# kan-bayashi/ParallelWaveGAN

Measured on AMD Instinct MI355X. Metric: HiFi-GAN V1 22.05 kHz generator inference RTF^-1 (audio samples/s), higher is better.
Workload: dtype f32; 1 GPU; HiFi-GAN V1 generator fwd, LJSpeech 22.05 kHz, B16 x 800 mel frames per GPU, fp32, random init; global_batch=16, parallelism=replicas x1

## Files before the change

### include/pwg_kernels.h

```cpp
#ifndef PWG_KERNELS_H_
#define PWG_KERNELS_H_

#include <stddef.h>
#include <stdint.h>

#ifdef __cplusplus
extern "C" {
#endif

typedef enum pwg_status {
  PWG_OK = 0,
  PWG_ERR_BAD_SHAPE = -1,
  PWG_ERR_UNSUPPORTED = -2,
  PWG_ERR_LAUNCH = -3,
  PWG_ERR_NULL = -4,
  PWG_ERR_WORKSPACE = -5
} pwg_status;

const char* pwg_last_error(void);
int pwg_abi_version(void);
int pwg_target_arch(void);

int pwg_prof_enable(int on);
int pwg_prof_reset(void);
// ... 72 lines not shown
int pwg_conv1d_num_tile_configs(void);
int pwg_conv1d_forward_cfg(const pwg_conv1d_desc* d, const float* x, const float* w_packed,
                           const float* bias, const float* add1, const float* add2, float* y,
                           int32_t tile_config, int32_t use_dma, void* stream);

int pwg_conv1d_bf16_supported(const pwg_conv1d_desc* d);
size_t pwg_conv1d_bf16_packed_weight_bytes(const pwg_conv1d_desc* d);
int pwg_conv1d_bf16_pack_weight(const pwg_conv1d_desc* d, const float* w, const float* scale, void* w_packed,
                                void* stream);
int pwg_conv1d_bf16_forward(const pwg_conv1d_desc* d, const float* x, const void* w_packed, const float* bias,
                            const float* add1, const float* add2, float* y, float* workspace, size_t workspace_floats,
                            void* stream);
int pwg_conv1d_bf16_forward_cfg(const pwg_conv1d_desc* d, const float* x, const void* w_packed, const float* bias,
                                const float* add1, const float* add2, float* y, int32_t mfma_shape, void* stream);

int pwg_conv1d_split_supported(const pwg_conv1d_desc* d);
size_t pwg_conv1d_split_packed_weight_bytes(const pwg_conv1d_desc* d);
int pwg_conv1d_split_pack_weight(const pwg_conv1d_desc* d, const float* w, const float* scale, void* w_packed,
                                 void* stream);
int pwg_conv1d_split_forward(const pwg_conv1d_desc* d, const float* x, const void* w_packed, const float* bias,
                             const float* add1, const float* add2, float* y, float* workspace, size_t workspace_floats,
                             void* stream);
int pwg_conv1d_split_forward_cfg(const pwg_conv1d_desc* d, const float* x, const void* w_packed, const float* bias,
                                 const float* add1, const float* add2, float* y, int32_t mfma_shape, int32_t tile_mode,
                                 void* stream);
int pwg_conv1d_split_step_form(const pwg_conv1d_desc* d);
int pwg_conv1d_split_forward_step(const pwg_conv1d_desc* d, const float* x, const void* w_packed, const float* bias,
                                  const float* add1, const float* add2, float* y, int32_t mfma_shape, int32_t tile_mode,
                                  int32_t step_form, void* stream);
int pwg_conv1d_split_window_form(const pwg_conv1d_desc* d);
int pwg_conv1d_split_forward_window(const pwg_conv1d_desc* d, const float* x, const void* w_packed, const float* bias,
                                    const float* add1, const float* add2, float* y, int32_t mfma_shape,
                                    int32_t tile_mode, int32_t step_form, int32_t window_form, void* stream);

int pwg_convtr1d_split_supported(const pwg_conv1d_desc* d);
size_t pwg_convtr1d_split_packed_weight_bytes(const pwg_conv1d_desc* d);
int pwg_convtr1d_split_pack_weight(const pwg_conv1d_desc* d, const float* w, const float* scale, void* w_packed,
                                   void* stream);
int pwg_convtr1d_split_forward(const pwg_conv1d_desc* d, const float* x, const void* w_packed, const float* bias,
                               const float* add1, const float* add2, float* y, float* workspace,
                               size_t workspace_floats, void* stream);
int pwg_convtr1d_split_forward_cfg(const pwg_conv1d_desc* d, const float* x, const void* w_packed, const float* bias,
                                   const float* add1, const float* add2, float* y, int32_t mfma_shape,
                                   int32_t tile_mode, void* stream);

int pwg_conv1d_stream_supported(const pwg_conv1d_desc* d);
size_t pwg_conv1d_stream_hist_floats(const pwg_conv1d_desc* d);
int pwg_conv1d_stream_forward(const pwg_conv1d_desc* d, const float* x, const float* hist_in, float* hist_out,
                              const float* w_packed, const float* bias, const float* add1, const float* add2, float* y,
                              void* stream);

int pwg_conv1d_stream_bf16_supported(const pwg_conv1d_desc* d);
int pwg_conv1d_stream_bf16_forward(const pwg_conv1d_desc* d, const float* x, const float* hist_in, float* hist_out,
                                   const void* w_packed_bf16, const float* bias, const float* add1,
                                   const float* add2, float* y, void* stream);

int pwg_conv1d_stream_delayed_supported(const pwg_conv1d_desc* d, int32_t delay1, int32_t delay2);
int pwg_conv1d_stream_delayed_forward(const pwg_conv1d_desc* d, const float* x, const float* hist_in, float* hist_out,
                                      const float* w_packed, const float* bias, const float* add1,
                                      const float* add1_hist_in, float* add1_hist_out, int32_t delay1, const float* add2,
                                      const float* add2_hist_in, float* add2_hist_out, int32_t delay2, int32_t valid_lo,
                                      int32_t valid_hi, float* y, void* stream);

int pwg_conv1d_stream_bf16_delayed_supported(const pwg_conv1d_desc* d, int32_t delay1, int32_t delay2);
int pwg_conv1d_stream_bf16_delayed_forward(const pwg_conv1d_desc* d, const float* x, const float* hist_in,
                                           float* hist_out, const void* w_packed_bf16, const float* bias,
// ... 359 lines not shown
```

### parallelwavegan_amd/_lib.py

```python
import ctypes
import os

_HERE = os.path.dirname(os.path.abspath(__file__))
LIB_PATH = os.environ.get("PWG_KERNEL_LIB") or os.path.join(_HERE, "libpwgkernels.so")

PWG_ACT_NONE, PWG_ACT_LEAKY_RELU, PWG_ACT_TANH, PWG_ACT_RELU = 0, 1, 2, 3
PWG_PAD_ZERO, PWG_PAD_REFLECT, PWG_PAD_REPLICATE = 0, 1, 2
ABI_VERSION = 15
SPECTRAL_NORM_SCRATCH_FLOATS = 257


class ConvDesc(ctypes.Structure):

    _fields_ = [
        ("batch", ctypes.c_int32),
        ("c_in", ctypes.c_int32),
        ("c_out", ctypes.c_int32),
        ("t_in", ctypes.c_int32),
        ("t_out", ctypes.c_int32),
        ("width", ctypes.c_int32),
        ("kernel", ctypes.c_int32),
        ("stride", ctypes.c_int32),
        ("dilation", ctypes.c_int32),
        ("pad_left", ctypes.c_int32),
# ... 82 lines not shown
    "pwg_target_arch": (ctypes.c_int, []),
    "pwg_debug_poison_lds": (ctypes.c_int, [ctypes.c_int]),
    "pwg_set_concurrency_hint": (ctypes.c_float, [ctypes.c_float]),
    "pwg_prof_enable": (ctypes.c_int, [ctypes.c_int]),
    "pwg_prof_reset": (ctypes.c_int, []),
    "pwg_prof_num_kernels": (ctypes.c_int, []),
    "pwg_prof_get": (ctypes.c_int, [_i32, ctypes.c_char_p, ctypes.c_size_t, ctypes.POINTER(ctypes.c_double),
                                    ctypes.POINTER(ctypes.c_int64), ctypes.POINTER(ctypes.c_double),
                                    ctypes.POINTER(ctypes.c_double)]),
    "pwg_conv1d_packed_weight_floats": (ctypes.c_size_t, [ctypes.POINTER(ConvDesc)]),
    "pwg_conv1d_pack_weight": (ctypes.c_int, [ctypes.POINTER(ConvDesc), _vp, _vp, _vp, _vp]),
    "pwg_conv1d_forward_workspace_floats": (ctypes.c_size_t, [ctypes.POINTER(ConvDesc)]),
    "pwg_conv1d_forward": (ctypes.c_int, [ctypes.POINTER(ConvDesc), _vp, _vp, _vp, _vp, _vp, _vp, _vp, ctypes.c_size_t,
                                          _vp]),
    "pwg_conv1d_bf16_supported": (ctypes.c_int, [ctypes.POINTER(ConvDesc)]),
    "pwg_conv1d_bf16_packed_weight_bytes": (ctypes.c_size_t, [ctypes.POINTER(ConvDesc)]),
    "pwg_conv1d_bf16_pack_weight": (ctypes.c_int, [ctypes.POINTER(ConvDesc), _vp, _vp, _vp, _vp]),
    "pwg_conv1d_bf16_forward": (ctypes.c_int, [ctypes.POINTER(ConvDesc), _vp, _vp, _vp, _vp, _vp, _vp, _vp, ctypes.c_size_t,
                                               _vp]),
    "pwg_conv1d_bf16_forward_cfg": (ctypes.c_int, [ctypes.POINTER(ConvDesc), _vp, _vp, _vp, _vp, _vp, _vp, _i32, _vp]),
    "pwg_conv1d_split_supported": (ctypes.c_int, [ctypes.POINTER(ConvDesc)]),
    "pwg_conv1d_split_packed_weight_bytes": (ctypes.c_size_t, [ctypes.POINTER(ConvDesc)]),
    "pwg_conv1d_split_pack_weight": (ctypes.c_int, [ctypes.POINTER(ConvDesc), _vp, _vp, _vp, _vp]),
    "pwg_conv1d_split_forward": (ctypes.c_int, [ctypes.POINTER(ConvDesc), _vp, _vp, _vp, _vp, _vp, _vp, _vp,
                                                ctypes.c_size_t, _vp]),
    "pwg_conv1d_split_forward_cfg": (ctypes.c_int, [ctypes.POINTER(ConvDesc), _vp, _vp, _vp, _vp, _vp, _vp, _i32, _i32,
                                                    _vp]),
    "pwg_conv1d_split_step_form": (ctypes.c_int, [ctypes.POINTER(ConvDesc)]),
    "pwg_conv1d_split_forward_step": (ctypes.c_int, [ctypes.POINTER(ConvDesc), _vp, _vp, _vp, _vp, _vp, _vp, _i32, _i32,
                                                     _i32, _vp]),
    "pwg_conv1d_split_window_form": (ctypes.c_int, [ctypes.POINTER(ConvDesc)]),
    "pwg_conv1d_split_forward_window": (ctypes.c_int, [ctypes.POINTER(ConvDesc), _vp, _vp, _vp, _vp, _vp, _vp, _i32,
                                                       _i32, _i32, _i32, _vp]),
    "pwg_convtr1d_split_supported": (ctypes.c_int, [ctypes.POINTER(ConvDesc)]),
    "pwg_convtr1d_split_packed_weight_bytes": (ctypes.c_size_t, [ctypes.POINTER(ConvDesc)]),
    "pwg_convtr1d_split_pack_weight": (ctypes.c_int, [ctypes.POINTER(ConvDesc), _vp, _vp, _vp, _vp]),
    "pwg_convtr1d_split_forward": (ctypes.c_int, [ctypes.POINTER(ConvDesc), _vp, _vp, _vp, _vp, _vp, _vp, _vp,
                                                  ctypes.c_size_t, _vp]),
    "pwg_convtr1d_split_forward_cfg": (ctypes.c_int, [ctypes.POINTER(ConvDesc), _vp, _vp, _vp, _vp, _vp, _vp, _i32, _i32,
                                                      _vp]),
    "pwg_conv1d_stream_supported": (ctypes.c_int, [ctypes.POINTER(ConvDesc)]),
    "pwg_conv1d_stream_hist_floats": (ctypes.c_size_t, [ctypes.POINTER(ConvDesc)]),
    "pwg_conv1d_stream_forward": (ctypes.c_int, [ctypes.POINTER(ConvDesc), _vp, _vp, _vp, _vp, _vp, _vp, _vp, _vp, _vp]),
    "pwg_conv1d_stream_bf16_supported": (ctypes.c_int, [ctypes.POINTER(ConvDesc)]),
    "pwg_conv1d_stream_bf16_forward": (ctypes.c_int, [ctypes.POINTER(ConvDesc), _vp, _vp, _vp, _vp, _vp, _vp, _vp, _vp,
                                                      _vp]),
    "pwg_conv1d_stream_delayed_supported": (ctypes.c_int, [ctypes.POINTER(ConvDesc), _i32, _i32]),
    "pwg_conv1d_stream_delayed_forward": (ctypes.c_int, [ctypes.POINTER(ConvDesc), _vp, _vp, _vp, _vp, _vp, _vp, _vp, _vp,
                                                         _i32, _vp, _vp, _vp, _i32, _i32, _i32, _vp, _vp]),
    "pwg_conv1d_stream_bf16_delayed_supported": (ctypes.c_int, [ctypes.POINTER(ConvDesc), _i32, _i32]),
    "pwg_conv1d_stream_bf16_delayed_forward": (ctypes.c_int, [ctypes.POINTER(ConvDesc), _vp, _vp, _vp, _vp, _vp, _vp, _vp,
                                                              _vp, _i32, _vp, _vp, _vp, _i32, _i32, _i32, _vp, _vp]),
    "pwg_conv1d_stream_slots_forward": (ctypes.c_int, [ctypes.POINTER(ConvDesc), _vp, _vp, _vp, _vp, _vp, _vp, _vp, _vp,
                                                       _i32, _vp, _vp, _vp, _i32, _vp, _i32, _i32, _vp, _vp]),
    "pwg_conv1d_stream_slots_forward_bf16": (ctypes.c_int, [ctypes.POINTER(ConvDesc), _vp, _vp, _vp, _vp, _vp, _vp, _vp,
                                                            _vp, _i32, _vp, _vp, _vp, _i32, _vp, _i32, _i32, _vp, _vp]),
    "pwg_conv1d_stream_mirrored_supported": (ctypes.c_int, [ctypes.POINTER(ConvDesc)]),
    "pwg_conv1d_stream_mirrored_forward": (ctypes.c_int, [ctypes.POINTER(ConvDesc), _vp, _vp, _vp, _vp, _vp, _vp, _i32,
                                                          _i32, _i32, _i32, _vp]),
    "pwg_conv1d_packed_weight_bwd_floats": (ctypes.c_size_t, [ctypes.POINTER(ConvDesc)]),
    "pwg_conv1d_pack_weight_bwd": (ctypes.c_int, [ctypes.POINTER(ConvDesc), _vp, _vp, _vp, _vp]),
    "pwg_weight_bank_table_bytes": (ctypes.c_size_t, [_i32]),
    "pwg_weight_bank_build": (ctypes.c_int, [ctypes.POINTER(BankItem), _i32, _vp, ctypes.c_size_t,
                                             ctypes.POINTER(ctypes.c_int32)]),
    "pwg_weight_bank_prepare": (ctypes.c_int, [_vp, ctypes.POINTER(ctypes.c_int32), _i32, _vp]),
    "pwg_conv1d_backward_data_workspace_floats": (ctypes.c_size_t, [ctypes.POINTER(ConvDesc)]),
# ... 177 lines not shown
```

### parallelwavegan_amd/csrc/conv1d_split.hip

```cpp
#include "mfma_conv.h"

namespace pwg {
namespace {

constexpr int PARTS = 3;

struct SplitArgs : MfmaConvArgs {
  int plane;
  long part_stride;
  float pre_mul;
  unsigned pre_mask;
  int wide_out;
};

static int split_geometry(const pwg_conv1d_desc* d, MfmaConvGeom* g) {
  return mfma_conv_geometry("conv1d_split", PARTS, false, d, g);
}

__device__ __forceinline__ float pre_activate(float v, float mul, unsigned mask) {
  const float n = __uint_as_float(__float_as_uint(v * mul) & mask);
  return v > 0.f ? v : n;
}

template <int NT, bool CHECKED>
// ... 7 lines not shown
    const int t = base + grp * 4;
    const float* __restrict__ src = xc + (size_t)(oct * 8) * a.t_in + t;
    if (!CHECKED) {
      if (grp < ngroups) {
#pragma unroll
        for (int j = 0; j < 8; ++j) st[it][j] = *reinterpret_cast<const f32x4*>(src + (size_t)j * a.t_in);
      }
    } else {
      const bool tin = grp < ngroups && t >= 0 && t < a.t_in;
#pragma unroll
      for (int j = 0; j < 8; ++j) {
        f32x4 v = {0.f, 0.f, 0.f, 0.f};
        if (tin && oct * 8 + j < c_left) v = *reinterpret_cast<const f32x4*>(src + (size_t)j * a.t_in);
        st[it][j] = v;
      }
    }
  }
#pragma unroll
  for (int it = 0; it < ITEMS; ++it) {
    const int idx = tid + it * 256, oct = idx & 3, grp = idx >> 2;
    if (grp < ngroups) {
#pragma unroll
      for (int e = 0; e < 4; ++e) {
        float v[8];
#pragma unroll
        for (int j = 0; j < 8; ++j) v[j] = pre_activate(st[it][j][e], a.pre_mul, a.pre_mask);
        split3_store<8>(v, xs + (grp * 4 + e) * kConvRow + oct * 8, a.plane);
        __builtin_amdgcn_sched_barrier(0);
      }
    }
  }
}

template <int TILE, int TM, int TN, bool WIDE, bool FULL>
__device__ __forceinline__ void split_epilogue(const SplitArgs& a, const typename Mfma<TILE>::acc_t (&acc)[TM][TN],
                                               int row0, int col0, size_t out_base) {
  constexpr int HL = 64 / TILE, NG = TILE * TILE / 64 / 4, NV = TN * NG;
  constexpr int NB = WIDE ? NV : 1, BATCHES = TM * NV / NB;
  const bool has_bias = a.bias != nullptr, has1 = a.add1 != nullptr, has2 = a.add2 != nullptr;
#pragma unroll
  for (int bi = 0; bi < BATCHES; ++bi) {
    const int mi = bi * NB / NV;
    const int m = row0 + mi * TILE, mc = FULL ? m : min(m, a.m - 1);
    const size_t row = out_base + (size_t)mc * a.t_out;
    int q[NB];
#pragma unroll
    for (int k = 0; k < NB; ++k) {
      const int n = (bi * NB + k) % NV;
      q[k] = col0 + (n / NG) * TILE + (n % NG) * (4 * HL);
    }
    auto load = [&](const float* __restrict__ src, f32x4 (&t)[NB]) {
#pragma unroll
      for (int k = 0; k < NB; ++k) {
        if (WIDE) {
          t[k] = *reinterpret_cast<const f32x4*>(src + row + (FULL ? q[k] : min(q[k], a.nq - 4)));
        } else {
#pragma unroll
          for (int e = 0; e < 4; ++e) t[k][e] = src[row + min(q[k] + e, a.nq - 1)];
        }
      }
    };
    f32x4 t1[NB], t2[NB], v[NB];
    float bias = 0.f;
    if (has_bias) bias = a.bias[mc];
    if (has1) load(a.add1, t1);
    if (has2) load(a.add2, t2);
#pragma unroll
    for (int k = 0; k < NB; ++k) {
      const int n = (bi * NB + k) % NV;
#pragma unroll
      for (int e = 0; e < 4; ++e) v[k][e] = acc[mi][n / NG][(n % NG) * 4 + e];
// ... 189 lines not shown
#pragma unroll
  for (int mi = 0; mi < TM; ++mi)
#pragma unroll
    for (int ni = 0; ni < TN; ++ni)
#pragma unroll
      for (int i = 0; i < NREG; ++i) acc[mi][ni][i] = 0.f;

  for (int chunk = 0; chunk < a.cin_chunks; ++chunk) {
    if (chunk) __syncthreads();
    stage_chunk<NT, VEC>(a, c, chunk, xs);
    __syncthreads();
#pragma unroll 1
    for (int s = 0; s < a.taps * KSTEPS; ++s) {
      const SplitStepId next = split_step_successor(step, a.cin_chunks, a.taps, KSTEPS);
      split_step_streamed<TILE, TM, TN, kConvRow, true>(
          wf, a.w, a.part_stride, wrow + split_step_rows<TILE>(a.cin_chunks, a.m_pad, step, c.h),
          wrow + split_step_rows<TILE>(a.cin_chunks, a.m_pad, next, c.h), xs,
          c.sh + c.wave_n * (WN * 32) + c.r + step.tap * a.dil, split_step_off<TILE>(step, c.h), a.plane, acc);
      step = next;
    }
  }

  const size_t out_base = (size_t)c.b * a.c_out * a.t_out;
  const int row0 = c.m0 + c.wave_m * (WM * 32) + c.r, col0 = c.q0 + c.wave_n * (WN * 32) + 4 * c.h;
  const bool full = c.m0 + MT <= a.m && c.q0 + NT <= a.nq;
  if (!a.wide_out)
    split_epilogue<TILE, TM, TN, false, false>(a, acc, row0, col0, out_base);
  else if (full)
    split_epilogue<TILE, TM, TN, true, true>(a, acc, row0, col0, out_base);
  else
    split_epilogue<TILE, TM, TN, true, false>(a, acc, row0, col0, out_base);
}

typedef __attribute__((address_space(3))) void* lds_ptr_t;

static inline size_t split_raw_bytes(int rows) { return (size_t)KC * rows * sizeof(float); }

__device__ __forceinline__ void request_raw_window(const float* __restrict__ xw, int t_in, int ngroups, float* raww,
                                                   int lane) {
  const int total = 8 * ngroups;
  const int dq = 64 / ngroups, dr = 64 - dq * ngroups;
  int j = lane / ngroups, g = lane - j * ngroups;
  for (int e0 = 0; e0 < total; e0 += 64) {
    if (e0 + lane < total)
      __builtin_amdgcn_global_load_lds(xw + (size_t)j * t_in + 4 * g, (lds_ptr_t)(raww + e0 * 4), 16, 0, 0);
    j += dq, g += dr;
    if (g >= ngroups) g -= ngroups, ++j;
  }
}

__device__ __forceinline__ void split_raw_window(const SplitArgs& a, const float* raww, int ngroups, __bf16* xs, int wave,
                                                 int lane) {
  for (int grp = lane; grp < ngroups; grp += 64) {
    f32x4 st[8];
#pragma unroll
    for (int j = 0; j < 8; ++j) st[j] = *reinterpret_cast<const f32x4*>(raww + (j * ngroups + grp) * 4);
#pragma unroll
    for (int e = 0; e < 4; ++e) {
      float v[8];
#pragma unroll
      for (int j = 0; j < 8; ++j) v[j] = pre_activate(st[j][e], a.pre_mul, a.pre_mask);
      split3_store<8>(v, xs + (grp * 4 + e) * kConvRow + wave * 8, a.plane);
      __builtin_amdgcn_sched_barrier(0);
    }
  }
}
// ... 79 lines not shown
  };
};

static void split_fill_args(SplitArgs* a, const pwg_conv1d_desc* d, const MfmaConvGeom& g, const MfmaConvPlan& p,
                            const float* x, const void* w_packed, const float* bias, const float* add1, const float* add2,
                            float* y) {
  mfma_conv_fill_args(a, d, g, x, w_packed, bias, add1, add2, y);
  a->plane = p.plane;
  a->part_stride = image_elems(g) / 8;
  a->pre_mul = d->pre_act == PWG_ACT_LEAKY_RELU ? d->pre_slope : (d->pre_act == PWG_ACT_RELU ? 0.0f : 1.0f);
  a->pre_mask = d->pre_act == PWG_ACT_RELU ? 0u : ~0u;
  a->wide_out = d->t_out % 4 == 0 && ((reinterpret_cast<uintptr_t>(y) | reinterpret_cast<uintptr_t>(add1) |
                                       reinterpret_cast<uintptr_t>(add2)) & 15u) == 0;
}

constexpr int kStepPlanDecides = 0, kStepResident = 1, kStepStreamed = 2;
constexpr int kStreamedMinTaps = 7, kStreamedMinChunks = 2;
static int split_step_form(const MfmaConvGeom& g) {
  if (!split_image_addressable(image_elems(g))) return kStepResident;
  return g.taps >= kStreamedMinTaps && g.cin_chunks >= kStreamedMinChunks ? kStepStreamed : kStepResident;
}

constexpr int kWindowPlanDecides = 0, kWindowStaged = 1, kWindowPrefetched = 2;
constexpr size_t kLdsPerCu = 160 * 1024, kWindowLdsShare = kLdsPerCu / 3;
constexpr int kWindowMaxTaps = 0;
static size_t split_window_lds(const MfmaConvPlan& p) { return p.lds + split_raw_bytes(p.plane / kConvRow); }
static bool split_window_covers(const MfmaConvPlan& p) { return p.vec && split_window_lds(p) <= kLdsPerCu; }
static int split_window_form(const MfmaConvGeom& g, const MfmaConvPlan& p) {
  if (!split_window_covers(p) || split_step_form(g) == kStepStreamed) return kWindowStaged;
  return g.taps <= kWindowMaxTaps && g.cin_chunks >= 2 && split_window_lds(p) <= kWindowLdsShare ? kWindowPrefetched
                                                                                                   : kWindowStaged;
}

static int split_forward(const pwg_conv1d_desc* d, const float* x, const void* w_packed, const float* bias,
                         const float* add1, const float* add2, float* y, int mfma_shape, int tile_mode, int step_form,
                         int window_form, hipStream_t stream) {
  MfmaConvGeom g;
  int rc = split_geometry(d, &g);
  if (rc != PWG_OK) return rc;
  PWG_REQUIRE(step_form >= kStepPlanDecides && step_form <= kStepStreamed, PWG_ERR_BAD_SHAPE,
              "conv1d_split: step_form = %d (0 = the plan decides, 1 = resident, 2 = streamed)", step_form);
  PWG_REQUIRE(window_form >= kWindowPlanDecides && window_form <= kWindowPrefetched, PWG_ERR_BAD_SHAPE,
              "conv1d_split: window_form = %d (0 = the plan decides, 1 = staged, 2 = prefetched)", window_form);
  rc = mfma_conv_check_forward("conv1d_split", d, x, w_packed, y, mfma_shape, tile_mode);
  if (rc != PWG_OK) return rc;
  const MfmaConvPlan p = mfma_conv_plan(d, g, PARTS, tile_mode, x, add1, add2);
  PWG_REQUIRE(step_form != kStepStreamed || split_image_addressable(image_elems(g)), PWG_ERR_UNSUPPORTED,
              "conv1d_split: weight image too large for the streamed step");
  PWG_REQUIRE(window_form != kWindowPrefetched || step_form != kStepStreamed, PWG_ERR_UNSUPPORTED,
              "conv1d_split: the prefetched window (window_form = 2) has no streamed step (step_form = 2)");
  PWG_REQUIRE(window_form != kWindowPrefetched || p.vec, PWG_ERR_UNSUPPORTED,
              "conv1d_split: the prefetched window (window_form = 2) needs 16-B staging: t_in %% 4 == 0, x 16-B aligned, "
              "a window of at most %d columns", 2 * p.nt);
  PWG_REQUIRE(window_form != kWindowPrefetched || split_window_covers(p), PWG_ERR_UNSUPPORTED,
              "conv1d_split: the prefetched window (window_form = 2) needs %zu B of LDS (> %zu)", split_window_lds(p),
              kLdsPerCu);
  const bool prefetched = window_form == kWindowPrefetched ||
                          (window_form == kWindowPlanDecides && step_form == kStepPlanDecides &&
                           split_window_form(g, p) == kWindowPrefetched);
  const bool streamed = !prefetched && (step_form == kStepPlanDecides ? split_step_form(g) : step_form) == kStepStreamed;
  SplitArgs a;
  split_fill_args(&a, d, g, p, x, w_packed, bias, add1, add2, y);
  if (prefetched) {
    const size_t lds = split_window_lds(p);
    void (*kern)(SplitArgs) = mfma_shape == 32 ? mfma_conv_tile_kernel<WindowFamily::K, 32, SplitArgs>(p)
                                               : mfma_conv_tile_kernel<WindowFamily::K, 16, SplitArgs>(p);
    if (lds > kConvMaxLds && !lds_limit_is_set(reinterpret_cast<const void*>(kern), lds)) {
      hipError_t e = hipFuncSetAttribute(reinterpret_cast<const void*>(kern), hipFuncAttributeMaxDynamicSharedMemorySize,
                                         (int)lds);
      PWG_REQUIRE(e == hipSuccess, PWG_ERR_LAUNCH, "conv1d_split: cannot raise LDS limit to %zu: %s", lds,
                  hipGetErrorString(e));
    }
    maybe_poison_lds(stream);
    ProfScope prof(stream, "conv1d_split_mfma_kernel", p.flops, p.bytes);
    hipLaunchKernelGGL(kern, p.grid, dim3(256), lds, stream, a);
    PWG_CHECK_LAUNCH("conv1d_split");
    return PWG_OK;
  }
  maybe_poison_lds(stream);
  ProfScope prof(stream, "conv1d_split_mfma_kernel", p.flops, p.bytes);
  if (p.vec) {
    if (streamed)
      mfma_conv_launch<Family<true, true>::K>(p, mfma_shape, a, stream);
    else
      mfma_conv_launch<Family<true, false>::K>(p, mfma_shape, a, stream);
  } else {
    if (streamed)
      mfma_conv_launch<Family<false, true>::K>(p, mfma_shape, a, stream);
    else
      mfma_conv_launch<Family<false, false>::K>(p, mfma_shape, a, stream);
  }
  PWG_CHECK_LAUNCH("conv1d_split");
  return PWG_OK;
}

// ... 217 lines not shown
}
}

using namespace pwg;

extern "C" int pwg_conv1d_split_supported(const pwg_conv1d_desc* d) {
  MfmaConvGeom g;
  return split_geometry(d, &g) == PWG_OK ? 1 : 0;
}

extern "C" size_t pwg_conv1d_split_packed_weight_bytes(const pwg_conv1d_desc* d) {
  MfmaConvGeom g;
  if (split_geometry(d, &g) != PWG_OK) return 0;
  return (size_t)PARTS * image_elems(g) * sizeof(__bf16);
}

extern "C" int pwg_conv1d_split_pack_weight(const pwg_conv1d_desc* d, const float* w, const float* scale, void* w_packed,
                                            void* stream) {
  MfmaConvGeom g;
  int rc = split_geometry(d, &g);
  if (rc != PWG_OK) return rc;
  PWG_REQUIRE(w && w_packed, PWG_ERR_NULL, "conv1d_split_pack_weight: NULL pointer");
  mfma_conv_pack<PARTS>(d, g, w, scale, w_packed, (hipStream_t)stream);
  PWG_CHECK_LAUNCH("conv1d_split_pack_weight");
  return PWG_OK;
}

extern "C" int pwg_conv1d_split_forward(const pwg_conv1d_desc* d, const float* x, const void* w_packed, const float* bias,
                                        const float* add1, const float* add2, float* y, float* workspace,
                                        size_t workspace_floats, void* stream) {
  (void)workspace;
  (void)workspace_floats;
  return split_forward(d, x, w_packed, bias, add1, add2, y, kDefaultMfmaShape, 0, kStepPlanDecides, kWindowPlanDecides,
                       (hipStream_t)stream);
}

extern "C" int pwg_conv1d_split_forward_cfg(const pwg_conv1d_desc* d, const float* x, const void* w_packed,
                                            const float* bias, const float* add1, const float* add2, float* y,
                                            int32_t mfma_shape, int32_t tile_mode, void* stream) {
  return split_forward(d, x, w_packed, bias, add1, add2, y, mfma_shape, tile_mode, kStepPlanDecides, kWindowPlanDecides,
                       (hipStream_t)stream);
}

extern "C" int pwg_conv1d_split_forward_step(const pwg_conv1d_desc* d, const float* x, const void* w_packed,
                                             const float* bias, const float* add1, const float* add2, float* y,
                                             int32_t mfma_shape, int32_t tile_mode, int32_t step_form, void* stream) {
  return split_forward(d, x, w_packed, bias, add1, add2, y, mfma_shape, tile_mode, step_form, kWindowPlanDecides,
                       (hipStream_t)stream);
}

extern "C" int pwg_conv1d_split_forward_window(const pwg_conv1d_desc* d, const float* x, const void* w_packed,
                                               const float* bias, const float* add1, const float* add2, float* y,
                                               int32_t mfma_shape, int32_t tile_mode, int32_t step_form,
                                               int32_t window_form, void* stream) {
  return split_forward(d, x, w_packed, bias, add1, add2, y, mfma_shape, tile_mode, step_form, window_form,
                       (hipStream_t)stream);
}

extern "C" int pwg_conv1d_split_window_form(const pwg_conv1d_desc* d) {
  MfmaConvGeom g;
  if (split_geometry(d, &g) != PWG_OK) return 0;
  return split_window_form(g, mfma_conv_plan(d, g, PARTS, 0, nullptr, nullptr, nullptr));
}

extern "C" int pwg_conv1d_split_step_form(const pwg_conv1d_desc* d) {
  MfmaConvGeom g;
  if (split_geometry(d, &g) != PWG_OK) return 0;
  return split_step_form(g);
}

extern "C" int pwg_convtr1d_split_supported(const pwg_conv1d_desc* d) {
  MfmaConvGeom g;
  return convtr_geometry(d, &g) == PWG_OK ? 1 : 0;
}

extern "C" size_t pwg_convtr1d_split_packed_weight_bytes(const pwg_conv1d_desc* d) {
  MfmaConvGeom g;
  if (convtr_geometry(d, &g) != PWG_OK) return 0;
  return (size_t)PARTS * image_elems(g) * sizeof(__bf16);
}

extern "C" int pwg_convtr1d_split_pack_weight(const pwg_conv1d_desc* d, const float* w, const float* scale, void* w_packed,
                                              void* stream) {
  MfmaConvGeom g;
  int rc = convtr_geometry(d, &g);
  if (rc != PWG_OK) return rc;
  PWG_REQUIRE(w && w_packed, PWG_ERR_NULL, "convtr1d_split_pack_weight: NULL pointer");
  mfma_conv_pack<PARTS>(d, g, w, scale, w_packed, (hipStream_t)stream);
  PWG_CHECK_LAUNCH("convtr1d_split_pack_weight");
// ... 17 lines not shown
```

### parallelwavegan_amd/csrc/mfma_conv.h

```cpp
#pragma once
#include "common.h"

#include "bf16_mfma.h"

#include <stdint.h>

namespace pwg {

constexpr int KC = 32;
constexpr int kConvRow = KC + 8;
constexpr size_t kConvMaxLds = 64 * 1024;
constexpr int kConvFillWorkgroups = 256;

static inline int plane_rows(int nt, int halo) { return round_up(nt + halo + 3, 4); }
static inline size_t conv_lds_bytes(int parts, int nt, int halo) {
  return (size_t)parts * plane_rows(nt, halo) * kConvRow * sizeof(__bf16);
}

constexpr int conv_row_tile(int m) { return m <= 32 ? 32 : (m <= 64 ? 64 : 128); }
constexpr int image_m_pad(int m) { return (m + conv_row_tile(m) - 1) / conv_row_tile(m) * conv_row_tile(m); }
constexpr int image_chunks(int c_in) { return (c_in + KC - 1) / KC; }

struct MfmaConvGeom {
  int taps, dil, x_off;
// ... 167 lines not shown
#pragma unroll
  for (int p = 0; p < 3; ++p) wf[p] = split_part_request(w, part_stride, row, p);
}

template <int TILE, int TM, int TN, int ROW, bool XFIRST>
__device__ __forceinline__ void split_step_streamed(bf16x8 (&wf)[3], const bf16x8* __restrict__ w, long part_stride,
                                                    unsigned row, unsigned row_next, const __bf16* xs, int col, int off,
                                                    int plane, typename Mfma<TILE>::acc_t (&acc)[TM][TN]) {
  bf16x8 bfr[3][TN];
  split_plane_fragments<TILE, TN, ROW>(bfr, xs, col, off, plane);
  static_assert(kSplitWeightPart[0] == 2 && kSplitWeightPart[1] != 2 && kSplitWeightPart[2] != 2 &&
                    kSplitWeightPart[3] != 2 && kSplitWeightPart[4] != 2 && kSplitWeightPart[5] != 2,
                "lo is read by the first product only");
#pragma unroll
  for (int mi = 0; mi < TM; ++mi) {
    const unsigned rn = mi + 1 < TM ? row + (mi + 1) * TILE : row_next;
    bf16x8 nx[3];
    nx[0] = split_part_request(w, part_stride, rn, 0);
    nx[1] = split_part_request(w, part_stride, rn, 1);
    __builtin_amdgcn_sched_barrier(0);
#pragma unroll
    for (int p = 0; p < 6; ++p) {
      split_product<TILE, TN, XFIRST>(p, wf, bfr, acc[mi]);
      if (p == 0) {
        __builtin_amdgcn_sched_barrier(0);
        nx[2] = split_part_request(w, part_stride, rn, 2);
        __builtin_amdgcn_sched_barrier(0);
      }
    }
#pragma unroll
    for (int p = 0; p < 3; ++p) wf[p] = nx[p];
    __builtin_amdgcn_sched_barrier(0);
  }
}

template <int PARTS>
static __global__ __launch_bounds__(256) void mfma_conv_pack_kernel(const float* __restrict__ w,
                                                                    const float* __restrict__ scale,
                                                                    __bf16* __restrict__ wp, int c_in, int c_out, int kernel,
                                                                    int taps, int cin_pad, int m, int m_pad, int phases,
                                                                    int transposed) {
  const long total = (long)taps * cin_pad * m_pad;
  for (long i = blockIdx.x * 256L + threadIdx.x; i < total; i += (long)gridDim.x * 256L) {
    const ImageIndex e = image_decode(i, cin_pad, m_pad);
    float v = 0.f;
    if (e.ci < c_in && e.row < m) {
      if (transposed) {
        const int co = e.row / phases, ph = e.row - co * phases;
        const int kk = e.tap == 0 ? ph + phases : ph;
        v = w[((long)e.ci * c_out + co) * kernel + kk];
        if (scale) v *= scale[e.ci];
      } else {
        v = w[((long)e.row * c_in + e.ci) * kernel + e.tap];
        if (scale) v *= scale[e.row];
      }
    }
    if (PARTS == 1) {
      wp[i] = (__bf16)v;
    } else {
      __bf16 hi, mid, lo;
      split3(v, hi, mid, lo);
      wp[i] = hi;
      wp[total + i] = mid;
      wp[2 * total + i] = lo;
    }
  }
// ... 116 lines not shown
```

### parallelwavegan_amd/ops.py

```python
import ctypes

import torch

from . import _lib
from ._lib import ConvDesc, ResUnitDesc, WaveNetDesc

ACT = {None: _lib.PWG_ACT_NONE, "none": _lib.PWG_ACT_NONE, "leaky_relu": _lib.PWG_ACT_LEAKY_RELU,
       "tanh": _lib.PWG_ACT_TANH, "relu": _lib.PWG_ACT_RELU}
PAD = {"zero": _lib.PWG_PAD_ZERO, "reflect": _lib.PWG_PAD_REFLECT, "replicate": _lib.PWG_PAD_REPLICATE}


PARAM_EPOCH = [0]


def bump_param_epoch():
    PARAM_EPOCH[0] += 1


def cache_epoch():
    return PARAM_EPOCH[0]


def param_epoch(p):
    return getattr(p, "_pwg_epoch", 0)
# ... 193 lines not shown
def conv1d_forward_bf16(desc, x, w_packed, bias=None, add1=None, add2=None, out=None, mfma_shape=None):
    return _conv1d_forward_mfma("bf16", desc, _zero_padded(desc), x, w_packed, bias, add1, add2, out,
                                None if mfma_shape is None else (int(mfma_shape),))


def conv1d_split_supported(desc):
    return bool(_lib.lib().pwg_conv1d_split_supported(ctypes.byref(desc)))


def pack_weight_split(desc, w, scale=None):
    return _pack_weight_mfma("split", desc, w, scale)


STEP_FORMS = {1: "resident", 2: "streamed"}


def conv1d_split_step_form(desc):
    form = _lib.lib().pwg_conv1d_split_step_form(ctypes.byref(desc))
    if form == 0:
        _lib.check(-1, "conv1d_split_step_form")
    return STEP_FORMS[form]


WINDOW_FORMS = {1: "staged", 2: "prefetched"}


def conv1d_split_window_form(desc):
    form = _lib.lib().pwg_conv1d_split_window_form(ctypes.byref(desc))
    if form == 0:
        _lib.check(-1, "conv1d_split_window_form")
    return WINDOW_FORMS[form]


def conv1d_forward_split(desc, x, w_packed, bias=None, add1=None, add2=None, out=None, mfma_shape=None, tile_mode=0,
                         step_form=0, window_form=0):
    if window_form:
        cfg = (int(mfma_shape or 16), int(tile_mode), int(step_form), int(window_form))
        return _conv1d_forward_mfma("split", desc, desc, x, w_packed, bias, add1, add2, out, cfg, entry="window")
    if step_form:
        cfg = (int(mfma_shape or 16), int(tile_mode), int(step_form))
        return _conv1d_forward_mfma("split", desc, desc, x, w_packed, bias, add1, add2, out, cfg, entry="step")
    cfg = None if mfma_shape is None and not tile_mode else (int(mfma_shape or 16), int(tile_mode))
    return _conv1d_forward_mfma("split", desc, desc, x, w_packed, bias, add1, add2, out, cfg)


def convtr1d_split_supported(desc):
    return bool(_lib.lib().pwg_convtr1d_split_supported(ctypes.byref(desc)))


def pack_weight_split_transposed(desc, w, scale=None):
    return _pack_weight_mfma("split", desc, w, scale, op="convtr1d")


def conv1d_forward_split_transposed(desc, x, w_packed, bias=None, add1=None, add2=None, out=None, mfma_shape=None,
                                    tile_mode=0):
    cfg = None if mfma_shape is None and not tile_mode else (int(mfma_shape or 16), int(tile_mode))
    return _conv1d_forward_mfma("split", desc, desc, x, w_packed, bias, add1, add2, out, cfg, op="convtr1d")


def conv1d_stream_supported(desc):
    return bool(_lib.lib().pwg_conv1d_stream_supported(ctypes.byref(desc)))


def conv1d_stream_hist_floats(desc):
    return _lib.lib().pwg_conv1d_stream_hist_floats(ctypes.byref(desc))


def _conv1d_stream_out(desc, x, hist_in, hist_out, add1, add2, out):
# ... 825 lines not shown
```

Before: 84.21 million samples/s.

## Add wide-wave MFMA split-conv tile for admitted conv classes

Adds a split-bf16 conv kernel variant where each wave covers a 32x128 output sub-tile (WM=1, WN=4) instead of the square layout, so each weight fragment is reused across four column tiles and the input plane fragments are prefetched one column ahead. The plan selects it automatically for two admitted shape classes (4 chunks/128 rows with 3 taps, and 8 chunks/256 rows with 7–11 taps) when the 128x128 workgroup tile and the default MFMA shape are used. The epilogue gains a batch-size parameter so the wide kernel stores in smaller batches. The kernel uses launch_bounds(256,3), which carries register-pressure and occupancy risk, and a public API entry point is added to force or query the tile form.

```diff
diff --git a/include/pwg_kernels.h b/include/pwg_kernels.h
--- a/include/pwg_kernels.h
+++ b/include/pwg_kernels.h
@@ -128,6 +128,10 @@
 int pwg_conv1d_split_forward_window(const pwg_conv1d_desc* d, const float* x, const void* w_packed, const float* bias,
                                     const float* add1, const float* add2, float* y, int32_t mfma_shape,
                                     int32_t tile_mode, int32_t step_form, int32_t window_form, void* stream);
+int pwg_conv1d_split_tile_form(const pwg_conv1d_desc* d);
+int pwg_conv1d_split_forward_tile(const pwg_conv1d_desc* d, const float* x, const void* w_packed, const float* bias,
+                                  const float* add1, const float* add2, float* y, int32_t mfma_shape, int32_t tile_mode,
+                                  int32_t step_form, int32_t window_form, int32_t tile_form, void* stream);
 
 int pwg_convtr1d_split_supported(const pwg_conv1d_desc* d);
 size_t pwg_convtr1d_split_packed_weight_bytes(const pwg_conv1d_desc* d);
diff --git a/parallelwavegan_amd/_lib.py b/parallelwavegan_amd/_lib.py
--- a/parallelwavegan_amd/_lib.py
+++ b/parallelwavegan_amd/_lib.py
@@ -138,6 +138,9 @@
     "pwg_conv1d_split_window_form": (ctypes.c_int, [ctypes.POINTER(ConvDesc)]),
     "pwg_conv1d_split_forward_window": (ctypes.c_int, [ctypes.POINTER(ConvDesc), _vp, _vp, _vp, _vp, _vp, _vp, _i32,
                                                        _i32, _i32, _i32, _vp]),
+    "pwg_conv1d_split_tile_form": (ctypes.c_int, [ctypes.POINTER(ConvDesc)]),
+    "pwg_conv1d_split_forward_tile": (ctypes.c_int, [ctypes.POINTER(ConvDesc), _vp, _vp, _vp, _vp, _vp, _vp, _i32, _i32,
+                                                     _i32, _i32, _i32, _vp]),
     "pwg_convtr1d_split_supported": (ctypes.c_int, [ctypes.POINTER(ConvDesc)]),
     "pwg_convtr1d_split_packed_weight_bytes": (ctypes.c_size_t, [ctypes.POINTER(ConvDesc)]),
     "pwg_convtr1d_split_pack_weight": (ctypes.c_int, [ctypes.POINTER(ConvDesc), _vp, _vp, _vp, _vp]),
diff --git a/parallelwavegan_amd/csrc/conv1d_split.hip b/parallelwavegan_amd/csrc/conv1d_split.hip
--- a/parallelwavegan_amd/csrc/conv1d_split.hip
+++ b/parallelwavegan_amd/csrc/conv1d_split.hip
@@ -63,11 +63,12 @@
   }
 }
 
-template <int TILE, int TM, int TN, bool WIDE, bool FULL>
+template <int TILE, int TM, int TN, bool WIDE, bool FULL, int BATCH = TN * (TILE * TILE / 64 / 4)>
 __device__ __forceinline__ void split_epilogue(const SplitArgs& a, const typename Mfma<TILE>::acc_t (&acc)[TM][TN],
                                                int row0, int col0, size_t out_base) {
   constexpr int HL = 64 / TILE, NG = TILE * TILE / 64 / 4, NV = TN * NG;
-  constexpr int NB = WIDE ? NV : 1, BATCHES = TM * NV / NB;
+  constexpr int NB = WIDE ? BATCH : 1, BATCHES = TM * NV / NB;
+  static_assert(NV % BATCH == 0, "a batch stays inside one mi");
   const bool has_bias = a.bias != nullptr, has1 = a.add1 != nullptr, has2 = a.add2 != nullptr;
 #pragma unroll
   for (int bi = 0; bi < BATCHES; ++bi) {
@@ -323,6 +324,64 @@
     split_epilogue<TILE, TM, TN, true, false>(a, acc, row0, col0, out_base);
 }
 
+template <int TILE, bool VEC>
+__global__ __launch_bounds__(256, 3) void conv1d_split_wide_mfma_kernel(SplitArgs a) {
+  constexpr int HL = 64 / TILE;
+  constexpr int KSTEPS = KC / (8 * HL);
+  constexpr int WAVES_M = 4, WM = 1, WN = 4;
+  constexpr int TM = WM * 32 / TILE, TN = WN * 32 / TILE;
+  constexpr int NREG = TILE * TILE / 64;
+  constexpr int MT = WAVES_M * WM * 32, NT = WN * 32;
+  constexpr int EPILOGUE_BATCH = 4;
+  typedef typename Mfma<TILE>::acc_t acc_t;
+
+  extern __shared__ __attribute__((aligned(16))) unsigned char smem[];
+  __bf16* xs = reinterpret_cast<__bf16*>(smem);
+
+  const MfmaConvTile c = mfma_conv_tile<TILE, MT, NT, WAVES_M, VEC>(a);
+
+  const unsigned wrow = c.m0 + c.wave_m * (WM * 32) + c.r;
+  bf16x8 wf[TM][3];
+  SplitStepId step{0, 0, 0};
+#pragma unroll
+  for (int mi = 0; mi < TM; ++mi)
+    split_step_request(wf[mi], a.w, a.part_stride,
+                       wrow + mi * TILE + split_step_rows<TILE>(a.cin_chunks, a.m_pad, step, c.h));
+
+  acc_t acc[TM][TN];
+#pragma unroll
+  for (int mi = 0; mi < TM; ++mi)
+#pragma unroll
+    for (int ni = 0; ni < TN; ++ni)
+#pragma unroll
+      for (int i = 0; i < NREG; ++i) acc[mi][ni][i] = 0.f;
+
+  for (int chunk = 0; chunk < a.cin_chunks; ++chunk) {
+    if (chunk) __syncthreads();
+    stage_chunk<NT, VEC>(a, c, chunk, xs);
+    __syncthreads();
+#pragma unroll 1
+    for (int s = 0; s < a.taps * KSTEPS; ++s) {
+      const SplitStepId next = split_step_successor(step, a.cin_chunks, a.taps, KSTEPS);
+      split_step_wide<TILE, TM, TN, kConvRow, true>(wf, a.w, a.part_stride,
+                                                    wrow + split_step_rows<TILE>(a.cin_chunks, a.m_pad, next, c.h), xs,
+                                                    c.sh + c.r + step.tap * a.dil, split_step_off<TILE>(step, c.h),
+                                                    a.plane, acc);
+      step = next;
+    }
+  }
+
+  const size_t out_base = (size_t)c.b * a.c_out * a.t_out;
+  const int row0 = c.m0 + c.wave_m * (WM * 32) + c.r, col0 = c.q0 + 4 * c.h;
+  const bool full = c.m0 + MT <= a.m && c.q0 + NT <= a.nq;
+  if (!a.wide_out)
+    split_epilogue<TILE, TM, TN, false, false>(a, acc, row0, col0, out_base);
+  else if (full)
+    split_epilogue<TILE, TM, TN, true, true, EPILOGUE_BATCH>(a, acc, row0, col0, out_base);
+  else
+    split_epilogue<TILE, TM, TN, true, false, EPILOGUE_BATCH>(a, acc, row0, col0, out_base);
+}
+
 typedef __attribute__((address_space(3))) void* lds_ptr_t;
 
 static inline size_t split_raw_bytes(int rows) { return (size_t)KC * rows * sizeof(float); }
@@ -468,12 +527,39 @@
                                                                                                    : kWindowStaged;
 }
 
+constexpr int kTilePlanDecides = 0, kTileSquare = 1, kTileWide = 2;
+struct WideClass {
+  int cin_chunks, m_pad, min_taps, max_taps;
+};
+constexpr WideClass kWideAdmitted[] = {{4, 128, 3, 3}, {8, 256, 7, 11}};
+static bool split_tile_covers(const MfmaConvGeom& g, const MfmaConvPlan& p) {
+  return !p.small && p.mt == 128 && p.nt == 128 && split_image_addressable(image_elems(g));
+}
+static int split_tile_form(const MfmaConvGeom& g, const MfmaConvPlan& p) {
+  if (!split_tile_covers(g, p)) return kTileSquare;
+  for (const WideClass& c : kWideAdmitted)
+    if (g.cin_chunks == c.cin_chunks && g.m_pad == c.m_pad && g.taps >= c.min_taps && g.taps <= c.max_taps)
+      return kTileWide;
+  return kTileSquare;
+}
+
+template <bool VEC>
+static void split_launch_wide(const MfmaConvPlan& p, const SplitArgs& a, hipStream_t stream) {
+  hipLaunchKernelGGL((conv1d_split_wide_mfma_kernel<16, VEC>), p.grid, dim3(256), p.lds, stream, a);
+}
+
 static int split_forward(const pwg_conv1d_desc* d, const float* x, const void* w_packed, const float* bias,
                          const float* add1, const float* add2, float* y, int mfma_shape, int tile_mode, int step_form,
-                         int window_form, hipStream_t stream) {
+                         int window_form, int tile_form, hipStream_t stream) {
   MfmaConvGeom g;
   int rc = split_geometry(d, &g);
   if (rc != PWG_OK) return rc;
+  PWG_REQUIRE(tile_form >= kTilePlanDecides && tile_form <= kTileWide, PWG_ERR_BAD_SHAPE,
+              "conv1d_split: tile_form = %d (0 = the plan decides, 1 = square, 2 = wide)", tile_form);
+  PWG_REQUIRE(tile_form != kTileWide || (step_form == kStepPlanDecides && window_form == kWindowPlanDecides),
+              PWG_ERR_UNSUPPORTED,
+              "conv1d_split: the wide tile (tile_form = 2) takes no step_form (%d) and no window_form (%d)", step_form,
+              window_form);
   PWG_REQUIRE(step_form >= kStepPlanDecides && step_form <= kStepStreamed, PWG_ERR_BAD_SHAPE,
               "conv1d_split: step_form = %d (0 = the plan decides, 1 = resident, 2 = streamed)", step_form);
   PWG_REQUIRE(window_form >= kWindowPlanDecides && window_form <= kWindowPrefetched, PWG_ERR_BAD_SHAPE,
@@ -495,8 +581,29 @@
                           (window_form == kWindowPlanDecides && step_form == kStepPlanDecides &&
                            split_window_form(g, p) == kWindowPrefetched);
   const bool streamed = !prefetched && (step_form == kStepPlanDecides ? split_step_form(g) : step_form) == kStepStreamed;
+  PWG_REQUIRE(tile_form != kTileWide || (!p.small && p.mt == 128 && p.nt == 128), PWG_ERR_UNSUPPORTED,
+              "conv1d_split: the wide tile (tile_form = 2) needs the 128 x 128 workgroup tile; this launch has %d x %d",
+              p.mt, p.nt);
+  PWG_REQUIRE(tile_form != kTileWide || split_image_addressable(image_elems(g)), PWG_ERR_UNSUPPORTED,
+              "conv1d_split: weight image too large for the wide tile");
+  PWG_REQUIRE(tile_form != kTileWide || mfma_shape == 16, PWG_ERR_UNSUPPORTED,
+              "conv1d_split: the wide tile (tile_form = 2) is built for mfma_shape 16 only (not %d)", mfma_shape);
+  const bool wide = tile_form == kTileWide ||
+                    (tile_form == kTilePlanDecides && step_form == kStepPlanDecides &&
+                     window_form == kWindowPlanDecides && !prefetched && mfma_shape == 16 &&
+                     split_tile_form(g, p) == kTileWide);
   SplitArgs a;
   split_fill_args(&a, d, g, p, x, w_packed, bias, add1, add2, y);
+  if (wide) {
+    maybe_poison_lds(stream);
+    ProfScope prof(stream, "conv1d_split_mfma_kernel", p.flops, p.bytes);
+    if (p.vec)
+      split_launch_wide<true>(p, a, stream);
+    else
+      split_launch_wide<false>(p, a, stream);
+    PWG_CHECK_LAUNCH("conv1d_split");
+    return PWG_OK;
+  }
   if (prefetched) {
     const size_t lds = split_window_lds(p);
     void (*kern)(SplitArgs) = mfma_shape == 32 ? mfma_conv_tile_kernel<WindowFamily::K, 32, SplitArgs>(p)
@@ -780,21 +887,21 @@
   (void)workspace;
   (void)workspace_floats;
   return split_forward(d, x, w_packed, bias, add1, add2, y, kDefaultMfmaShape, 0, kStepPlanDecides, kWindowPlanDecides,
-                       (hipStream_t)stream);
+                       kTilePlanDecides, (hipStream_t)stream);
 }
 
 extern "C" int pwg_conv1d_split_forward_cfg(const pwg_conv1d_desc* d, const float* x, const void* w_packed,
                                             const float* bias, const float* add1, const float* add2, float* y,
                                             int32_t mfma_shape, int32_t tile_mode, void* stream) {
   return split_forward(d, x, w_packed, bias, add1, add2, y, mfma_shape, tile_mode, kStepPlanDecides, kWindowPlanDecides,
-                       (hipStream_t)stream);
+                       kTilePlanDecides, (hipStream_t)stream);
 }
 
 extern "C" int pwg_conv1d_split_forward_step(const pwg_conv1d_desc* d, const float* x, const void* w_packed,
                                              const float* bias, const float* add1, const float* add2, float* y,
                                              int32_t mfma_shape, int32_t tile_mode, int32_t step_form, void* stream) {
   return split_forward(d, x, w_packed, bias, add1, add2, y, mfma_shape, tile_mode, step_form, kWindowPlanDecides,
-                       (hipStream_t)stream);
+                       kTilePlanDecides, (hipStream_t)stream);
 }
 
 extern "C" int pwg_conv1d_split_forward_window(const pwg_conv1d_desc* d, const float* x, const void* w_packed,
@@ -802,7 +909,21 @@
                                                int32_t mfma_shape, int32_t tile_mode, int32_t step_form,
                                                int32_t window_form, void* stream) {
   return split_forward(d, x, w_packed, bias, add1, add2, y, mfma_shape, tile_mode, step_form, window_form,
+                       kTilePlanDecides, (hipStream_t)stream);
+}
+
+extern "C" int pwg_conv1d_split_forward_tile(const pwg_conv1d_desc* d, const float* x, const void* w_packed,
+                                             const float* bias, const float* add1, const float* add2, float* y,
+                                             int32_t mfma_shape, int32_t tile_mode, int32_t step_form,
+                                             int32_t window_form, int32_t tile_form, void* stream) {
+  return split_forward(d, x, w_packed, bias, add1, add2, y, mfma_shape, tile_mode, step_form, window_form, tile_form,
                        (hipStream_t)stream);
+}
+
+extern "C" int pwg_conv1d_split_tile_form(const pwg_conv1d_desc* d) {
+  MfmaConvGeom g;
+  if (split_geometry(d, &g) != PWG_OK) return 0;
+  return split_tile_form(g, mfma_conv_plan(d, g, PARTS, 0, nullptr, nullptr, nullptr));
 }
 
 extern "C" int pwg_conv1d_split_window_form(const pwg_conv1d_desc* d) {
diff --git a/parallelwavegan_amd/csrc/mfma_conv.h b/parallelwavegan_amd/csrc/mfma_conv.h
--- a/parallelwavegan_amd/csrc/mfma_conv.h
+++ b/parallelwavegan_amd/csrc/mfma_conv.h
@@ -223,6 +223,38 @@
     for (int p = 0; p < 3; ++p) wf[p] = nx[p];
     __builtin_amdgcn_sched_barrier(0);
   }
+}
+
+template <int TILE, int TM, int TN, int ROW, bool XFIRST>
+__device__ __forceinline__ void split_step_wide(bf16x8 (&wf)[TM][3], const bf16x8* __restrict__ w, long part_stride,
+                                                unsigned row_next, const __bf16* xs, int col, int off, int plane,
+                                                typename Mfma<TILE>::acc_t (&acc)[TM][TN]) {
+  typedef typename Mfma<TILE>::acc_t acc_t;
+  bf16x8 nx[TM][3], cur[3][1];
+#pragma unroll
+  for (int mi = 0; mi < TM; ++mi) split_step_request(nx[mi], w, part_stride, row_next + mi * TILE);
+  split_plane_fragments<TILE, 1, ROW>(cur, xs, col, off, plane);
+  __builtin_amdgcn_sched_barrier(0);
+#pragma unroll
+  for (int ni = 0; ni < TN; ++ni) {
+    bf16x8 ahead[3][1];
+    if (ni + 1 < TN) split_plane_fragments<TILE, 1, ROW>(ahead, xs, col + (ni + 1) * TILE, off, plane);
+    __builtin_amdgcn_sched_barrier(0);
+#pragma unroll
+    for (int p = 0; p < 6; ++p)
+#pragma unroll
+      for (int mi = 0; mi < TM; ++mi)
+        split_product<TILE, 1, XFIRST>(p, wf[mi], cur, reinterpret_cast<acc_t(&)[1]>(acc[mi][ni]));
+    if (ni + 1 < TN) {
+#pragma unroll
+      for (int p = 0; p < 3; ++p) cur[p][0] = ahead[p][0];
+    }
+    __builtin_amdgcn_sched_barrier(0);
+  }
+#pragma unroll
+  for (int mi = 0; mi < TM; ++mi)
+#pragma unroll
+    for (int p = 0; p < 3; ++p) wf[mi][p] = nx[mi][p];
 }
 
 template <int PARTS>
diff --git a/parallelwavegan_amd/ops.py b/parallelwavegan_amd/ops.py
--- a/parallelwavegan_amd/ops.py
+++ b/parallelwavegan_amd/ops.py
@@ -249,8 +249,21 @@
     return WINDOW_FORMS[form]
 
 
+TILE_FORMS = {1: "square", 2: "wide"}
+
+
+def conv1d_split_tile_form(desc):
+    form = _lib.lib().pwg_conv1d_split_tile_form(ctypes.byref(desc))
+    if form == 0:
+        _lib.check(-1, "conv1d_split_tile_form")
+    return TILE_FORMS[form]
+
+
 def conv1d_forward_split(desc, x, w_packed, bias=None, add1=None, add2=None, out=None, mfma_shape=None, tile_mode=0,
-                         step_form=0, window_form=0):
+                         step_form=0, window_form=0, tile_form=0):
+    if tile_form:
+        cfg = (int(mfma_shape or 16), int(tile_mode), int(step_form), int(window_form), int(tile_form))
+        return _conv1d_forward_mfma("split", desc, desc, x, w_packed, bias, add1, add2, out, cfg, entry="tile")
     if window_form:
         cfg = (int(mfma_shape or 16), int(tile_mode), int(step_form), int(window_form))
         return _conv1d_forward_mfma("split", desc, desc, x, w_packed, bias, add1, add2, out, cfg, entry="window")
```

Result: no change. 84.54 million samples/s (median of 6 runs) (+0.4%).
